# meta-pytorch/torchx

Measured on AMD Instinct MI355X. Metric: tokens_per_second, higher is better.
Workload: dtype bf16; 1 GPU; model=llama3_8b, global_batch=4, seq_len=4096, parallelism=dp1

## Files before the change

torchx_amd/ops/__init__.py:

```python

from __future__ import annotations

import importlib.util
import math
from pathlib import Path
from typing import Optional, Tuple

import torch

from . import reference

_SO = Path(__file__).resolve().parent / "_hip_ops.so"
_hip = None
_load_err: Optional[str] = None


def _load():
    global _hip, _load_err
    if _hip is not None:
        return _hip
    if not _SO.exists():
        _load_err = f"{_SO} not built (run torchx_amd/ops/build.py)"
        return None
    try:
# ... 144 lines not shown
        T, H = x2.shape
        dx = torch.empty_like(x2)
        single = T <= chunk
        dw_acc = None if single else torch.zeros_like(w, dtype=torch.float32)
        loss_sum = torch.zeros((), device=x2.device, dtype=torch.float32)
        inv_t = 1.0 / T
        gscale = torch.full((min(chunk, T),), inv_t, device=x2.device,
                            dtype=torch.float32)
        wt = (hip.transpose_bf16(w)
              if w.shape[0] % 64 == 0 and w.shape[1] % 64 == 0 else None)
        for s in range(0, T, chunk):
            e = min(T, s + chunk)
            x_c = x2[s:e]
            t_c = targets[s:e].contiguous()
            logits_c = x_c @ w.t()
            loss_c, lse_c = hip.ce_fwd(logits_c, t_c)
            loss_sum += loss_c.sum()
            dlog_c = hip.ce_bwd(logits_c, t_c, lse_c, gscale[:e - s])
            if wt is not None:
                torch.matmul(dlog_c, wt.t(), out=dx[s:e])
            else:
                torch.matmul(dlog_c, w, out=dx[s:e])
            if single:
                dw_acc = dlog_c.t() @ x_c
            else:
                dw_acc += dlog_c.t() @ x_c
        ctx.save_for_backward(dx, dw_acc)
        return loss_sum * inv_t

    @staticmethod
    def backward(ctx, gout: torch.Tensor):
        dx, dw_acc = ctx.saved_tensors
        if dw_acc.dtype == dx.dtype:
            dw = dw_acc * gout.to(dx.dtype)
        else:
            dw = (dw_acc * gout.to(torch.float32)).to(dx.dtype)
        dx = dx * gout.to(dx.dtype)
        return dx, dw, None, None


def fused_linear_cross_entropy(
    x: torch.Tensor, w: torch.Tensor, targets: torch.Tensor,
    chunk: int = 16384,
) -> torch.Tensor:
    H = x.shape[-1]
    x2 = x.reshape(-1, H)
    t = targets.reshape(-1)
    if _on_gpu(x):
        if torch.is_grad_enabled() and (x.requires_grad or w.requires_grad):
            return _FusedLinearCE.apply(x2.contiguous(), w, t, chunk)
        hip = hip_ops()
        x2 = x2.contiguous()
        T = x2.shape[0]
        loss_sum = torch.zeros((), device=x.device, dtype=torch.float32)
        for s in range(0, T, chunk):
            e = min(T, s + chunk)
            loss_c, _ = hip.ce_fwd(x2[s:e] @ w.t(), t[s:e].contiguous())
            loss_sum += loss_c.sum()
        return loss_sum / T
    return reference.cross_entropy(x2 @ w.t(), t)




class _FlashAttention(torch.autograd.Function):
    @staticmethod
    def forward(ctx, q: torch.Tensor, k: torch.Tensor, v: torch.Tensor,
                causal: bool, scale: float):
        o, lse = hip_ops().attn_fwd(
            q.contiguous(), k.contiguous(), v.contiguous(), scale, causal
        )
        ctx.save_for_backward(q, k, v, o, lse)
        ctx.causal = causal
        ctx.scale = scale
        return o

    @staticmethod
    def backward(ctx, dout: torch.Tensor):
        q, k, v, o, lse = ctx.saved_tensors
        dq, dk, dv = hip_ops().attn_bwd(
            q, k, v, o, dout.contiguous(), lse, ctx.scale, ctx.causal
        )
        return dq, dk, dv, None, None


def flash_attention(
    q: torch.Tensor, k: torch.Tensor, v: torch.Tensor,
    causal: bool = True, scale: Optional[float] = None,
) -> torch.Tensor:
    if scale is None:
        scale = 1.0 / math.sqrt(q.shape[-1])
    if _on_gpu(q):
        return _FlashAttention.apply(q, k, v, causal, scale)
    return reference.attention(q, k, v, causal=causal, scale=scale)




def adamw_step(
    p32: torch.Tensor, p16: torch.Tensor, grad: torch.Tensor,
    m: torch.Tensor, v: torch.Tensor, *, lr: float, beta1: float = 0.9,
    beta2: float = 0.95, eps: float = 1e-8, weight_decay: float = 0.1,
    step: int = 1,
) -> None:
    if p32.is_cuda:
        hip_ops().adamw_step(p32, p16, grad, m, v, lr, beta1, beta2, eps,
                             weight_decay, step)
    else:
        reference.adamw_step(p32, p16, grad, m, v, lr=lr, beta1=beta1,
                             beta2=beta2, eps=eps, weight_decay=weight_decay,
                             step=step)


def mfma_probe(a: torch.Tensor, b: torch.Tensor) -> torch.Tensor:
    return hip_ops().mfma_probe(a, b)




class _FastLinear(torch.autograd.Function):
    @staticmethod
    def forward(ctx, x: torch.Tensor, w: torch.Tensor):
        ctx.save_for_backward(x, w)
        return x @ w.t()

    @staticmethod
    def backward(ctx, dy: torch.Tensor):
        x, w = ctx.saved_tensors
        hip = hip_ops()
        wt = hip.transpose_bf16(w)
        dy2 = dy.reshape(-1, dy.shape[-1]).contiguous()
        x2 = x.reshape(-1, x.shape[-1])
        dx = (dy2 @ wt.t()).view_as(x)
        M, N = dy2.shape
        via_t = N <= 8192 and M % 64 == 0 and N % 64 == 0
        wg = w.grad if w.is_leaf else None
        if wg is not None and wg.is_contiguous():
            a = hip.transpose_bf16(dy2) if via_t else dy2.t()
            if getattr(w, "_wgrad_fresh", False):
                torch.matmul(a, x2, out=wg)
                w._wgrad_fresh = False
            else:
                wg.addmm_(a, x2)
            from torchx_amd.parallel.ddp import grad_ready

            grad_ready(w)
            return dx, None
        dw = (hip.transpose_bf16(dy2) @ x2) if via_t else (dy2.t() @ x2)
        return dx, dw


def fast_linear(x: torch.Tensor, w: torch.Tensor) -> torch.Tensor:
    if (x.is_cuda and w.dtype == torch.bfloat16
            and w.shape[0] % 64 == 0 and w.shape[1] % 64 == 0):
        return _FastLinear.apply(x, w)
    return torch.nn.functional.linear(x, w)




class _FusedAttentionQKV(torch.autograd.Function):
    @staticmethod
    def forward(ctx, qkv: torch.Tensor, cos: torch.Tensor, sin: torch.Tensor,
                Hq: int, Hkv: int, causal: bool, scale: float):
        hip = hip_ops()
        roped = hip.rope_qkv(qkv.contiguous(), cos, sin, Hq, Hkv, 1.0, False)
# ... 153 lines not shown
```

torchx_amd/ops/csrc/attention.hip:

```cpp
#include "common.h"

typedef __bf16 mbf16x8 __attribute__((ext_vector_type(8)));

#define HD 128
#define QBLK 32
#define KBLK 32
#define NWAVES 4
#define BLOCK_Q (QBLK * NWAVES)
#define BLOCK_K (KBLK * NWAVES)

__device__ __forceinline__ f32x16 mfma32(mbf16x8 a, mbf16x8 b, f32x16 c) {
  return __builtin_amdgcn_mfma_f32_32x32x16_bf16(a, b, c, 0, 0, 0);
}

__device__ __forceinline__ unsigned int pack_bf16x2(float a, float b) {
  unsigned int r;
  asm("v_cvt_pk_bf16_f32 %0, %1, %2" : "=v"(r) : "v"(a), "v"(b));
  return r;
}

__device__ __forceinline__ int c_row(int r, int half) {
  return (r & 3) + 8 * (r >> 2) + 4 * half;
}

// ... 301 lines not shown
      #pragma unroll
      for (int r = 0; r < 32; ++r) {
        sv[r] = __builtin_amdgcn_exp2f(sv[r] - m_run);
        row_sum += sv[r];
      }
      row_sum += __shfl_xor(row_sum, 32, 64);
      l_run += row_sum;

      mbf16x8 pf[4];
      cvals_to_frags(sv, hi, &pf[0], &pf[1]);
      cvals_to_frags(sv + 16, hi, &pf[2], &pf[3]);

      __builtin_amdgcn_s_setprio(1);
      #pragma unroll
      for (int dt = 0; dt < 4; ++dt) {
        #pragma unroll
        for (int ks = 0; ks < 4; ++ks) {
          acc_o[dt] = mfma32(nat_tr_frag(vcur, ks, dt), pf[ks], acc_o[dt]);
        }
      }
      __builtin_amdgcn_s_setprio(0);
    }

    if (has_next) {
      asm volatile("s_waitcnt vmcnt(0)");
      __syncthreads();
      char* tk = k0; k0 = k1; k1 = tk;
      char* tv = vcur; vcur = vnxt; vnxt = tv;
    }
  }

  if (!wave_active || q_row >= S) return;

  const float inv_l = (l_run > 0.f) ? 1.0f / l_run : 0.f;
  unsigned short* ob =
      o + (((long)b * S + q_row) * Hq + hq) * HD;
  #pragma unroll
  for (int dt = 0; dt < 4; ++dt) {
    #pragma unroll
    for (int g = 0; g < 4; ++g) {
      bf16x4_raw w;
      #pragma unroll
      for (int j = 0; j < 4; ++j) {
        w[j] = (short)f32_to_bf16(acc_o[dt][4 * g + j] * inv_l);
      }
      *(bf16x4_raw*)(ob + dt * 32 + 8 * g + 4 * (hi ? 1 : 0)) = w;
    }
  }
  if (!hi) {
    lse[((long)b * Hq + hq) * S + q_row] = (m_run + __log2f(l_run)) * LN2;
  }
}

__global__ void __launch_bounds__(256)
attn_bwd_pre_kernel(const unsigned short* __restrict__ dout,
                    const unsigned short* __restrict__ o,
                    float* __restrict__ delta,
                    long rows,
                    int S, int Hq) {
  const long row = (long)blockIdx.x * 16 + threadIdx.x / 16;
  if (row >= rows) return;
  const int sl = threadIdx.x & 15;
  const unsigned short* dp = dout + row * HD + sl * 8;
  const unsigned short* op = o + row * HD + sl * 8;
  ushort8 dv = *(const ushort8*)dp;
  ushort8 ov = *(const ushort8*)op;
  float acc = 0.f;
  #pragma unroll
  for (int j = 0; j < 8; ++j) {
    acc = fmaf(bf16_to_f32(dv[j]), bf16_to_f32(ov[j]), acc);
  }
  #pragma unroll
  for (int off = 8; off >= 1; off >>= 1) {
    acc += __shfl_down(acc, off, 16);
  }
  if (sl == 0) {
    const long b = row / ((long)S * Hq);
    const long s = (row / Hq) % S;
    const long h = row % Hq;
    delta[(b * Hq + h) * S + s] = acc;
  }
}

template <int TFKV>
__global__ void __launch_bounds__(256, 2)
attn_bwd_dq_kernel(const unsigned short* __restrict__ q,
                   const unsigned short* __restrict__ k,
                   const unsigned short* __restrict__ v,
                   const unsigned short* __restrict__ dout,
                   const float* __restrict__ lse,
                   const float* __restrict__ delta,
                   unsigned short* __restrict__ dq,
                   int B, int S, int Hq, int Hkv, float scale, int causal,
                   long q_rs, long kv_rs, long dq_rs) {
  __shared__ __align__(16) char smem[4 * (TFKV * 256)];
  char* kcur = smem;
  char* knxt = smem + TFKV * 256;
  char* vcur = smem + 2 * (TFKV * 256);
  char* vnxt = smem + 3 * (TFKV * 256);

  const int nqt = (S + BLOCK_Q - 1) / BLOCK_Q;
  const int G = Hq / Hkv;
  int b, hq, qt;
  map_block_fwd(B, Hq, Hkv, nqt, G, &b, &hq, &qt);
  const int hkv = hq / G;

  const int wave = threadIdx.x / 64;
  const int lane = threadIdx.x & 63;
  const bool hi = lane >= 32;
  const int qr = lane & 31;

  const long q_seq_stride = q_rs;
  const long kv_seq_stride = kv_rs;
  const unsigned short* qb = q + (long)b * S * q_seq_stride + (long)hq * HD;
  const unsigned short* kb = k + (long)b * S * kv_seq_stride + (long)hkv * HD;
  const unsigned short* vb = v + (long)b * S * kv_seq_stride + (long)hkv * HD;
  const unsigned short* dob =
      dout + ((long)b * S) * ((long)Hq * HD) + (long)hq * HD;

  const int q0_blk = qt * BLOCK_Q;
  const int qw0 = q0_blk + wave * QBLK;
  const long q_row = qw0 + qr;
  const bool wave_active = qw0 < S;
  const bool row_valid = q_row < S;

  mbf16x8 qfrag[8];
  float my_lse2 = 0.f, my_delta = 0.f;
  const long qrow_safe = row_valid ? q_row : (S - 1);
  const unsigned short* dop =
      dob + qrow_safe * ((long)Hq * HD) + (hi ? 8 : 0);
  {
    const unsigned short* qp = qb + qrow_safe * q_seq_stride + (hi ? 8 : 0);
    #pragma unroll
    for (int c = 0; c < 8; ++c) {
      qfrag[c] = __builtin_bit_cast(mbf16x8, *(const ushort8*)(qp + c * 16));
    }
    if (row_valid) {
      my_lse2 = lse[((long)b * Hq + hq) * S + q_row] * LOG2E;
      my_delta = delta[((long)b * Hq + hq) * S + q_row];
    }
  }

  f32x16 acc_dq[4] = {};
  const float sc2 = scale * LOG2E;

  const int kv_limit = causal ? min(S, q0_blk + BLOCK_Q) : S;
  const int ntiles = (kv_limit + TFKV - 1) / TFKV;
  const int qw_max = min(qw0 + QBLK - 1, S - 1);

  stage_k_glds<4, TFKV>(kb, 0, kv_seq_stride, S, kcur);
  stage_k_glds<4, TFKV>(vb, 0, kv_seq_stride, S, vcur);
  asm volatile("s_waitcnt vmcnt(0)");
  __syncthreads();

  for (int t = 0; t < ntiles; ++t) {
    const int kv0 = t * TFKV;
    const bool has_next = (t + 1) < ntiles;
    if (has_next) {
      stage_k_glds<4, TFKV>(kb, kv0 + TFKV, kv_seq_stride, S, knxt);
      stage_k_glds<4, TFKV>(vb, kv0 + TFKV, kv_seq_stride, S, vnxt);
    }

    const bool needed = wave_active && (!causal || kv0 <= qw_max);
    if (needed) {
      mbf16x8 dofrag[8];
      #pragma unroll
      for (int c = 0; c < 8; ++c) {
        dofrag[c] =
            __builtin_bit_cast(mbf16x8, *(const ushort8*)(dop + c * 16));
      }
      #pragma clang loop unroll(disable)
      for (int sb = 0; sb < TFKV / 32; ++sb) {
        if (causal && kv0 + 32 * sb > qw_max) break;
        f32x16 acc_s = {}, acc_dp = {};
        #pragma unroll
        for (int c = 0; c < 8; ++c) {
          acc_s = mfma32(kimg_frag(kcur, sb, c), qfrag[c], acc_s);
          acc_dp = mfma32(kimg_frag(vcur, sb, c), dofrag[c], acc_dp);
        }
        const int k0 = kv0 + 32 * sb;
        const bool mask_tile =
            (causal && k0 + 31 > qw0) || (k0 + 32 > S) || !row_valid;
        float ds[16];
        #pragma unroll
        for (int r = 0; r < 16; ++r) {
          float s2 = acc_s[r] * sc2;
          if (mask_tile) {
            const long kg = k0 + c_row(r, hi);
            if (kg >= S || !row_valid || (causal && kg > q_row)) {
              s2 = -3.0e38f;
            }
          }
          const float pr = __builtin_amdgcn_exp2f(s2 - my_lse2);
          ds[r] = scale * pr * (acc_dp[r] - my_delta);
        }
        mbf16x8 df0, df1;
        cvals_to_frags(ds, hi, &df0, &df1);
        #pragma unroll
        for (int dt = 0; dt < 4; ++dt) {
          acc_dq[dt] =
              mfma32(nat_tr_frag(kcur, 2 * sb, dt), df0, acc_dq[dt]);
          acc_dq[dt] =
              mfma32(nat_tr_frag(kcur, 2 * sb + 1, dt), df1, acc_dq[dt]);
        }
      }
    }

    if (has_next) {
      asm volatile("s_waitcnt vmcnt(0)");
      __syncthreads();
      char* tk = kcur; kcur = knxt; knxt = tk;
      char* tv = vcur; vcur = vnxt; vnxt = tv;
    }
  }

  if (!wave_active || !row_valid) return;
  unsigned short* dqb =
      dq + ((long)b * S + q_row) * dq_rs + (long)hq * HD;
  #pragma unroll
  for (int dt = 0; dt < 4; ++dt) {
    #pragma unroll
    for (int g = 0; g < 4; ++g) {
      bf16x4_raw w;
      #pragma unroll
      for (int j = 0; j < 4; ++j) {
        w[j] = (short)f32_to_bf16(acc_dq[dt][4 * g + j]);
      }
      *(bf16x4_raw*)(dqb + dt * 32 + 8 * g + 4 * (hi ? 1 : 0)) = w;
    }
  }
}

template <int TFKV = FKV>
__device__ __forceinline__ void stage_k_glds8(
    const unsigned short* __restrict__ kb, long kv0, long stride_elems,
    int S, char* kimg) {
  const int wave = threadIdx.x / 64;
  const int lane = threadIdx.x & 63;
  #pragma unroll
  for (int j = 0; j < TFKV / 32; ++j) {
    const int i = wave * (TFKV / 32) + j;
    const int row = i * 4 + (lane >> 4);
    const int colbyte = ((lane & 15) * 16) ^ ((row & 15) << 4);
    long srow = kv0 + row;
    if (srow >= S) srow = S - 1;
    const char* src = (const char*)(kb + srow * stride_elems) + colbyte;
    __builtin_amdgcn_global_load_lds(
        (const __attribute__((address_space(1))) unsigned int*)src,
        (__attribute__((address_space(3))) unsigned int*)(kimg + i * 1024),
        16, 0, 0);
  }
}


__device__ __forceinline__ void lds_nat_to_tr_own8(const char* nat,
                                                   char* tr_img) {
  const int wave = threadIdx.x / 64;
  const int lane = threadIdx.x & 63;
  #pragma unroll
  for (int pp = 0; pp < 2; ++pp) {
    const int c = wave * 128 + pp * 64 + lane;
    const int r = c >> 4, g = c & 15;
    const ushort8 v = *(const ushort8*)(
        nat + r * 256 + ((g * 16) ^ ((r & 15) << 4)));
    #pragma unroll
    for (int j = 0; j < 8; ++j) {
      const int d = 8 * g + j;
      const int gr = ((r >> 3) + vrot(d)) & 7;
      *(unsigned short*)(tr_img + d * 128 + gr * 16 + (r & 7) * 2) = v[j];
    }
  }
}

template <int TFKV>
__global__ void __launch_bounds__(512, 2)
attn_bwd_dkv_kernel(const unsigned short* __restrict__ q,
                    const unsigned short* __restrict__ k,
                    const unsigned short* __restrict__ v,
                    const unsigned short* __restrict__ dout,
                    const float* __restrict__ lse,
                    const float* __restrict__ delta,
                    unsigned short* __restrict__ dk,
                    unsigned short* __restrict__ dv,
                    int B, int S, int Hq, int Hkv, float scale, int causal,
                    long q_rs, long kv_rs, long dout_rs, long out_rs) {
  __shared__ __align__(16) char smem[4 * (TFKV * 256)];
  __shared__ float lse_buf[2][TFKV], del_buf[2][TFKV];
  char* qn_c = smem;
  char* don_c = smem + TFKV * 256;
  char* qn_n = smem + 2 * (TFKV * 256);
  char* don_n = smem + 3 * (TFKV * 256);

  const int nkt = (S + BLOCK_K - 1) / BLOCK_K;
  const int G = Hq / Hkv;
  int b, hkv, kt;
  {
    int bid = blockIdx.x;
    if (((B * Hkv) & 7) == 0) {
      const int xcd = bid & 7, slot = bid >> 3;
      const int g = (slot / nkt) * 8 + xcd;
      b = g / Hkv;
      hkv = g % Hkv;
      kt = slot % nkt;
    } else {
      b = bid / (Hkv * nkt);
      bid -= b * Hkv * nkt;
      hkv = bid / nkt;
      kt = bid % nkt;
    }
  }

  const int wave = threadIdx.x / 64;
  const bool is_dk = wave >= 4;
  const int lane = threadIdx.x & 63;
  const bool hi = lane >= 32;
  const int kr = lane & 31;

  const long q_seq_stride = q_rs;
  const long kv_seq_stride = kv_rs;
  const unsigned short* kb = k + (long)b * S * kv_seq_stride + (long)hkv * HD;
  const unsigned short* vb = v + (long)b * S * kv_seq_stride + (long)hkv * HD;

  const int kv0_blk = kt * BLOCK_K;
  const int kw0 = kv0_blk + (wave & 3) * KBLK;
  const long k_row = kw0 + kr;
  const bool wave_active = kw0 < S;
  const bool krow_valid = k_row < S;

  mbf16x8 kfrag[8], vfrag[8];
  {
    const long row = krow_valid ? k_row : (S - 1);
    const unsigned short* kp = kb + row * kv_seq_stride + (hi ? 8 : 0);
    const unsigned short* vp = vb + row * kv_seq_stride + (hi ? 8 : 0);
    #pragma unroll
    for (int c = 0; c < 8; ++c) {
      kfrag[c] = __builtin_bit_cast(mbf16x8, *(const ushort8*)(kp + c * 16));
      if (is_dk) {
        vfrag[c] =
            __builtin_bit_cast(mbf16x8, *(const ushort8*)(vp + c * 16));
      }
    }
  }

  f32x16 acc[4] = {};
  const float sc2 = scale * LOG2E;

  const int t0 = causal ? (kv0_blk / TFKV) : 0;
  const int nt = (S + TFKV - 1) / TFKV;
  const int nt_eff = nt - t0;
  const int total = G * nt_eff;

  auto head_q = [&](int gh) {
    return q + (long)b * S * q_seq_stride + (long)(hkv * G + gh) * HD;
  };
  auto head_do = [&](int gh) {
    return dout + (long)b * S * dout_rs + (long)(hkv * G + gh) * HD;
  };
  auto stage_lse = [&](int gh, int t, int buf) {
    const int hq_ = hkv * G + gh;
    const int q0_ = t * TFKV;
    if (threadIdx.x < TFKV) {
      const float* lse_b = lse + ((long)b * Hq + hq_) * S;
      const int qg = q0_ + threadIdx.x;
      lse_buf[buf][threadIdx.x] = (qg < S) ? lse_b[qg] * LOG2E : 0.f;
    } else if (threadIdx.x < 2 * TFKV) {
      const float* del_b = delta + ((long)b * Hq + hq_) * S;
      const int qg = q0_ + (threadIdx.x - TFKV);
      del_buf[buf][threadIdx.x - TFKV] = (qg < S) ? del_b[qg] : 0.f;
    }
  };

  stage_k_glds8<TFKV>(head_q(0), (long)t0 * TFKV, q_seq_stride, S, qn_c);
  stage_k_glds8<TFKV>(head_do(0), (long)t0 * TFKV, dout_rs, S, don_c);
  asm volatile("s_waitcnt vmcnt(0)");
  stage_lse(0, t0, 0);
  __syncthreads();

  const float* lse_cur = lse_buf[0];
  const float* del_cur = del_buf[0];
  int lse_nxt = 1;
  for (int idx = 0; idx < total; ++idx) {
    const int gh = idx / nt_eff;
    const int t = t0 + idx % nt_eff;
    const int q0 = t * TFKV;
    const int hq = hkv * G + gh;
    const bool has_next = (idx + 1) < total;
    const int ngh = (idx + 1) / nt_eff;
    const long nrow0 = (long)(t0 + (idx + 1) % nt_eff) * TFKV;
    if (has_next) {
      stage_k_glds8<TFKV>(head_q(ngh), nrow0, q_seq_stride, S, qn_n);
      stage_k_glds8<TFKV>(head_do(ngh), nrow0, dout_rs, S, don_n);
    }

    const bool needed =
        wave_active && (!causal || q0 + TFKV - 1 >= kw0);
    if (needed) {
      #pragma clang loop unroll(disable)
      for (int sb = 0; sb < TFKV / 32; ++sb) {
        if (causal && q0 + 32 * sb + 32 <= kw0) continue;
        f32x16 acc_s = {}, acc_dp = {};
        #pragma unroll
        for (int c = 0; c < 8; ++c) {
          acc_s = mfma32(kimg_frag(qn_c, sb, c), kfrag[c], acc_s);
          if (is_dk) {
            acc_dp = mfma32(kimg_frag(don_c, sb, c), vfrag[c], acc_dp);
          }
        }

        const int qs0 = q0 + 32 * sb;
        const bool mask_tile = (causal && qs0 < kw0 + 32)
                               || (qs0 + 32 > S) || !krow_valid;
        float cv[16];
        #pragma unroll
        for (int r = 0; r < 16; ++r) {
          const int ql = 32 * sb + c_row(r, hi);
          float s2 = acc_s[r] * sc2;
          if (mask_tile) {
            const long qg = q0 + ql;
            if (qg >= S || !krow_valid || (causal && k_row > qg)) {
              s2 = -3.0e38f;
            }
          }
          const float pr =
              __builtin_amdgcn_exp2f(s2 - lse_cur[ql]);
          cv[r] = is_dk ? scale * pr * (acc_dp[r] - del_cur[ql]) : pr;
        }

        mbf16x8 f0, f1;
        cvals_to_frags(cv, hi, &f0, &f1);

        const char* acc_img = is_dk ? qn_c : don_c;
        #pragma unroll
        for (int dt = 0; dt < 4; ++dt) {
          acc[dt] =
              mfma32(f0, nat_tr_frag(acc_img, 2 * sb, dt), acc[dt]);
          acc[dt] =
              mfma32(f1, nat_tr_frag(acc_img, 2 * sb + 1, dt), acc[dt]);
        }
      }
    }

    if (has_next) {
      asm volatile("s_waitcnt vmcnt(0)");
      stage_lse(ngh, t0 + (idx + 1) % nt_eff, lse_nxt);
      __syncthreads();
      lse_cur = lse_buf[lse_nxt];
      del_cur = del_buf[lse_nxt];
      lse_nxt ^= 1;
      char* tp;
      tp = qn_c; qn_c = qn_n; qn_n = tp;
      tp = don_c; don_c = don_n; don_n = tp;
    }
  }

  unsigned short* out = is_dk ? dk : dv;
  __syncthreads();
  float* tr = (float*)smem + wave * (32 * 36);
  if (wave_active) {
    #pragma unroll
    for (int dt = 0; dt < 4; ++dt) {
      __syncthreads();
      #pragma unroll
      for (int r = 0; r < 16; ++r) {
        tr[c_row(r, hi) * 36 + kr] = acc[dt][r];
      }
      __syncthreads();
      #pragma unroll
      for (int rep = 0; rep < 4; ++rep) {
        const int kk = kr;
        const int d0 = (hi ? 16 : 0) + rep * 4;
        if (kw0 + kk < S) {
          bf16x4_raw w;
          #pragma unroll
          for (int j = 0; j < 4; ++j) {
            w[j] = (short)f32_to_bf16(tr[kk * 36 + d0 + j]);
          }
          *(bf16x4_raw*)(out + ((long)b * S + kw0 + kk) * out_rs +
                         (long)hkv * HD + dt * 32 + d0) = w;
        }
      }
    }
  } else {
    #pragma unroll
    for (int i = 0; i < 8; ++i) __syncthreads();
  }
}

extern "C" void attn_fwd_launch(const void* q, const void* k, const void* v,
                                void* o, void* lse, int B, int S, int Hq,
                                int Hkv, float scale, int causal,
                                long q_rs, long kv_rs, hipStream_t stream) {
  static int fwd8 = -1;
  if (fwd8 < 0) {
    const char* e = getenv("TORCHX_AMD_FWD_8WAVE");
    fwd8 = (e && atoi(e)) ? 1 : 0;
  }
  if (fwd8 == 1) {
    const int nqt = (S + 8 * QBLK - 1) / (8 * QBLK);
    hipLaunchKernelGGL((attn_fwd_kernel<8>), dim3(B * Hq * nqt), dim3(512),
                       0, stream, (const unsigned short*)q,
                       (const unsigned short*)k, (const unsigned short*)v,
                       (unsigned short*)o, (float*)lse, B, S, Hq, Hkv,
                       scale, causal, q_rs, kv_rs);
  } else {
    const int nqt = (S + 4 * QBLK - 1) / (4 * QBLK);
    hipLaunchKernelGGL((attn_fwd_kernel<4>), dim3(B * Hq * nqt), dim3(256),
                       0, stream, (const unsigned short*)q,
                       (const unsigned short*)k, (const unsigned short*)v,
                       (unsigned short*)o, (float*)lse, B, S, Hq, Hkv,
                       scale, causal, q_rs, kv_rs);
  }
}

extern "C" void attn_bwd_launch(const void* q, const void* k, const void* v,
                                const void* o, const void* dout,
                                const void* lse, void* delta, void* dq,
                                void* dk, void* dv, int B, int S, int Hq,
                                int Hkv, float scale, int causal,
                                long q_rs, long kv_rs, long dqkv_q_rs,
                                long dqkv_kv_rs, hipStream_t stream) {
  const long rows = (long)B * S * Hq;
  hipLaunchKernelGGL(attn_bwd_pre_kernel, dim3((int)((rows + 15) / 16)),
                     dim3(256), 0, stream, (const unsigned short*)dout,
                     (const unsigned short*)o, (float*)delta, rows, S, Hq);
  const int nqt = (S + BLOCK_Q - 1) / BLOCK_Q;
  static int dq_fkv = -1;
  if (dq_fkv < 0) {
    const char* e = getenv("TORCHX_AMD_DQ_FKV");
    dq_fkv = (e && atoi(e) == 128) ? 128 : 64;
  }
  if (dq_fkv == 128 && S % 128 == 0) {
    hipLaunchKernelGGL((attn_bwd_dq_kernel<128>), dim3(B * Hq * nqt),
                       dim3(256), 0, stream, (const unsigned short*)q,
                       (const unsigned short*)k, (const unsigned short*)v,
                       (const unsigned short*)dout, (const float*)lse,
                       (const float*)delta, (unsigned short*)dq, B, S, Hq,
                       Hkv, scale, causal, q_rs, kv_rs, dqkv_q_rs);
  } else {
    hipLaunchKernelGGL((attn_bwd_dq_kernel<64>), dim3(B * Hq * nqt),
                       dim3(256), 0, stream, (const unsigned short*)q,
                       (const unsigned short*)k, (const unsigned short*)v,
                       (const unsigned short*)dout, (const float*)lse,
                       (const float*)delta, (unsigned short*)dq, B, S, Hq,
                       Hkv, scale, causal, q_rs, kv_rs, dqkv_q_rs);
  }
  const int nkt = (S + BLOCK_K - 1) / BLOCK_K;
  const long dout_rs = (long)Hq * HD;
  static int dkv_fkv = -1;
  if (dkv_fkv < 0) {
    const char* e = getenv("TORCHX_AMD_DKV_FKV");
    dkv_fkv = (e && atoi(e) == 64) ? 64 : 128;
  }
  if (dkv_fkv == 128 && S % 128 == 0) {
    hipLaunchKernelGGL((attn_bwd_dkv_kernel<128>), dim3(B * Hkv * nkt),
                       dim3(512), 0, stream, (const unsigned short*)q,
                       (const unsigned short*)k, (const unsigned short*)v,
                       (const unsigned short*)dout, (const float*)lse,
                       (const float*)delta, (unsigned short*)dk,
                       (unsigned short*)dv, B, S, Hq, Hkv,
                       scale, causal, q_rs, kv_rs, dout_rs, dqkv_kv_rs);
  } else {
    hipLaunchKernelGGL((attn_bwd_dkv_kernel<64>), dim3(B * Hkv * nkt),
                       dim3(512), 0, stream, (const unsigned short*)q,
                       (const unsigned short*)k, (const unsigned short*)v,
                       (const unsigned short*)dout, (const float*)lse,
                       (const float*)delta, (unsigned short*)dk,
                       (unsigned short*)dv, B, S, Hq, Hkv,
                       scale, causal, q_rs, kv_rs, dout_rs, dqkv_kv_rs);
  }
}
```

torchx_amd/ops/csrc/bindings.cpp:

```cpp
#include <torch/extension.h>
#include <c10/hip/HIPStream.h>

#include <hip/hip_runtime.h>

extern "C" {
void rope_launch(const void*, void*, const void*, const void*, long, int, int,
                 int, float, hipStream_t);
void swiglu_fwd_launch(const void*, const void*, void*, long, hipStream_t);
void swiglu_bwd_launch(const void*, const void*, const void*, void*, void*,
                       long, hipStream_t);
void rmsnorm_fwd_launch(const void*, const void*, void*, void*, long, int,
                        float, hipStream_t);
void rmsnorm_bwd_launch(const void*, const void*, const void*, const void*,
                        void*, void*, void*, long, int, hipStream_t);
long rmsnorm_bwd_dw_chunks(long);
void adamw_launch(void*, void*, const void*, void*, void*, long, float, float,
                  float, float, float, float, float, hipStream_t);
void ce_fwd_launch(const void*, const void*, void*, void*, long, int,
                   hipStream_t);
void ce_bwd_launch(const void*, const void*, const void*, const void*, void*,
                   long, int, hipStream_t);
void attn_fwd_launch(const void*, const void*, const void*, void*, void*, int,
                     int, int, int, float, int, long, long, hipStream_t);
void attn_bwd_launch(const void*, const void*, const void*, const void*,
                     const void*, const void*, void*, void*, void*, void*,
                     int, int, int, int, float, int, long, long, long, long,
                     hipStream_t);
void rope_qkv_launch(const void*, void*, const void*, const void*, long, int,
                     long, int, float, hipStream_t);
void swiglu_gu_fwd_launch(const void*, void*, long, long, hipStream_t);
void swiglu_gu_bwd_launch(const void*, const void*, void*, long, long,
                          hipStream_t);
void mfma_probe_launch(const void*, const void*, void*, hipStream_t);
void mfma_probe_tr_launch(const void*, const void*, void*, void*,
                          hipStream_t);
void fp8_cast_transpose_launch(const void*, void*, void*, void*,
                               const void*, long, long, int, hipStream_t);
void transpose_bf16_launch(const void*, void*, long, long, hipStream_t);
void decode_attn_launch(const void*, const void*, const void*, void*,
                        const void*, int, int, int, int, int, int, float,
                        hipStream_t);
void gemv_bf16_launch(const void*, const void*, void*, int, int, int,
                      hipStream_t);
void decode_attn_split_launch(const void*, const void*, const void*, void*,
                              void*, void*, const void*, int, int, int, int,
                              int, int, int, float, hipStream_t);
void decode_rope_cache_launch(const void*, void*, void*, void*, const void*,
                              const void*, const void*, int, int, int, int,
                              int, int, hipStream_t);
void rmsnorm_res_launch(const void*, const void*, const void*, void*, void*,
                        long, int, float, hipStream_t);
void gemv_swiglu_launch(const void*, const void*, void*, int, int, int,
                        hipStream_t);
}

namespace {

hipStream_t cur_stream() {
  return c10::hip::getCurrentHIPStream().stream();
}

void check_bf16(const at::Tensor& t, const char* name) {
  TORCH_CHECK(t.is_cuda(), name, " must be on GPU");
  TORCH_CHECK(t.scalar_type() == at::kBFloat16, name, " must be bf16");
  TORCH_CHECK(t.is_contiguous(), name, " must be contiguous");
}

void check_f32(const at::Tensor& t, const char* name) {
  TORCH_CHECK(t.is_cuda(), name, " must be on GPU");
  TORCH_CHECK(t.scalar_type() == at::kFloat, name, " must be f32");
  TORCH_CHECK(t.is_contiguous(), name, " must be contiguous");
}

}

std::vector<at::Tensor> rmsnorm_fwd(at::Tensor x, at::Tensor w, double eps) {
  check_bf16(x, "x");
  check_bf16(w, "w");
  const long H = x.size(-1);
  TORCH_CHECK(H % 2048 == 0 && H <= 8192, "rmsnorm: H must be k*2048, <=8192");
  const long rows = x.numel() / H;
  auto y = at::empty_like(x);
  auto invrms = at::empty({rows}, x.options().dtype(at::kFloat));
  rmsnorm_fwd_launch(x.data_ptr(), w.data_ptr(), y.data_ptr(),
                     invrms.data_ptr(), rows, (int)H, (float)eps,
                     cur_stream());
  return {y, invrms};
}

std::vector<at::Tensor> rmsnorm_bwd(at::Tensor dy, at::Tensor x, at::Tensor w,
                                    at::Tensor invrms) {
  check_bf16(dy, "dy");
  check_bf16(x, "x");
  const long H = x.size(-1);
  TORCH_CHECK(H % 2048 == 0 && H <= 8192, "rmsnorm: H must be k*2048, <=8192");
  const long rows = x.numel() / H;
  auto dx = at::empty_like(x);
  auto dw = at::empty({H}, x.options().dtype(at::kFloat));
  auto dw_part = at::empty({rmsnorm_bwd_dw_chunks(rows), H}, dw.options());
  rmsnorm_bwd_launch(dy.data_ptr(), x.data_ptr(), w.data_ptr(),
                     invrms.data_ptr(), dx.data_ptr(), dw.data_ptr(),
                     dw_part.data_ptr(), rows, (int)H, cur_stream());
  return {dx, dw};
}

at::Tensor rope(at::Tensor x, at::Tensor cos_t, at::Tensor sin_t, long heads,
                double sign) {
  check_bf16(x, "x");
  check_f32(cos_t, "cos");
  check_f32(sin_t, "sin");
// ... 4 lines not shown
  auto y = at::empty_like(x);
  rope_launch(x.data_ptr(), y.data_ptr(), cos_t.data_ptr(), sin_t.data_ptr(),
              rows, (int)D, (int)heads, (int)S, (float)sign, cur_stream());
  return y;
}

at::Tensor swiglu_fwd(at::Tensor g, at::Tensor u) {
  check_bf16(g, "g");
  check_bf16(u, "u");
  auto out = at::empty_like(g);
  swiglu_fwd_launch(g.data_ptr(), u.data_ptr(), out.data_ptr(), g.numel(),
                    cur_stream());
  return out;
}

std::vector<at::Tensor> swiglu_bwd(at::Tensor dout, at::Tensor g,
                                   at::Tensor u) {
  check_bf16(dout, "dout");
  auto dg = at::empty_like(g);
  auto du = at::empty_like(u);
  swiglu_bwd_launch(dout.data_ptr(), g.data_ptr(), u.data_ptr(), dg.data_ptr(),
                    du.data_ptr(), g.numel(), cur_stream());
  return {dg, du};
}

void adamw_step(at::Tensor p32, at::Tensor p16, at::Tensor g, at::Tensor m,
                at::Tensor v, double lr, double beta1, double beta2,
                double eps, double wd, long step) {
  check_f32(p32, "p32");
  check_bf16(p16, "p16");
  check_bf16(g, "g");
  const long n = p32.numel();
  TORCH_CHECK(n % 4 == 0, "adamw: n must be a multiple of 4");
  const float bc1 = 1.0f - powf((float)beta1, (float)step);
  const float bc2 = 1.0f - powf((float)beta2, (float)step);
  adamw_launch(p32.data_ptr(), p16.data_ptr(), g.data_ptr(), m.data_ptr(),
               v.data_ptr(), n, (float)lr, (float)beta1, (float)beta2,
               (float)eps, (float)wd, bc1, bc2, cur_stream());
}

std::vector<at::Tensor> ce_fwd(at::Tensor logits, at::Tensor targets) {
  check_bf16(logits, "logits");
  TORCH_CHECK(targets.scalar_type() == at::kLong, "targets must be int64");
  const long V = logits.size(-1);
  const long T = logits.numel() / V;
  auto loss = at::empty({T}, logits.options().dtype(at::kFloat));
  auto lse = at::empty({T}, logits.options().dtype(at::kFloat));
  ce_fwd_launch(logits.data_ptr(), targets.data_ptr(), loss.data_ptr(),
                lse.data_ptr(), T, (int)V, cur_stream());
  return {loss, lse};
}

at::Tensor ce_bwd(at::Tensor logits, at::Tensor targets, at::Tensor lse,
                  at::Tensor gscale) {
  check_bf16(logits, "logits");
  check_f32(lse, "lse");
  check_f32(gscale, "gscale");
  const long V = logits.size(-1);
  const long T = logits.numel() / V;
  auto dlogits = at::empty_like(logits);
  ce_bwd_launch(logits.data_ptr(), targets.data_ptr(), lse.data_ptr(),
                gscale.data_ptr(), dlogits.data_ptr(), T, (int)V,
                cur_stream());
  return dlogits;
}

std::vector<at::Tensor> attn_fwd(at::Tensor q, at::Tensor k, at::Tensor v,
                                 double scale, bool causal) {
  check_bf16(q, "q");
  check_bf16(k, "k");
  check_bf16(v, "v");
  const int B = q.size(0), S = q.size(1), Hq = q.size(2), D = q.size(3);
  const int Hkv = k.size(2);
  TORCH_CHECK(D == 128, "attention: head_dim must be 128");
  TORCH_CHECK(Hq % Hkv == 0, "attention: Hq must be a multiple of Hkv");
  auto o = at::empty_like(q);
  auto lse = at::empty({B, Hq, S}, q.options().dtype(at::kFloat));
  attn_fwd_launch(q.data_ptr(), k.data_ptr(), v.data_ptr(), o.data_ptr(),
                  lse.data_ptr(), B, S, Hq, Hkv, (float)scale, causal ? 1 : 0,
                  (long)Hq * 128, (long)Hkv * 128, cur_stream());
  return {o, lse};
}

std::vector<at::Tensor> attn_bwd(at::Tensor q, at::Tensor k, at::Tensor v,
                                 at::Tensor o, at::Tensor dout, at::Tensor lse,
                                 double scale, bool causal) {
  check_bf16(dout, "dout");
  const int B = q.size(0), S = q.size(1), Hq = q.size(2);
  const int Hkv = k.size(2);
  auto dq = at::empty_like(q);
  auto dk = at::empty_like(k);
  auto dv = at::empty_like(v);
  auto delta = at::empty({B, Hq, S}, q.options().dtype(at::kFloat));
  attn_bwd_launch(q.data_ptr(), k.data_ptr(), v.data_ptr(), o.data_ptr(),
                  dout.data_ptr(), lse.data_ptr(), delta.data_ptr(),
                  dq.data_ptr(), dk.data_ptr(), dv.data_ptr(), B, S, Hq, Hkv,
                  (float)scale, causal ? 1 : 0, (long)Hq * 128,
                  (long)Hkv * 128, (long)Hq * 128, (long)Hkv * 128,
                  cur_stream());
  return {dq, dk, dv};
}

std::vector<at::Tensor> attn_fwd_qkv(at::Tensor qkv, long Hq, long Hkv,
                                     double scale, bool causal) {
  check_bf16(qkv, "qkv");
  const int B = qkv.size(0), S = qkv.size(1);
  const long rs = (Hq + 2 * Hkv) * 128;
  TORCH_CHECK(qkv.size(2) == rs, "qkv last dim mismatch");
  auto o = at::empty({B, S, Hq, 128}, qkv.options());
  auto lse = at::empty({B, Hq, S}, qkv.options().dtype(at::kFloat));
  const unsigned short* base = (const unsigned short*)qkv.data_ptr();
  attn_fwd_launch(base, base + Hq * 128, base + (Hq + Hkv) * 128,
                  o.data_ptr(), lse.data_ptr(), B, S, (int)Hq, (int)Hkv,
                  (float)scale, causal ? 1 : 0, rs, rs, cur_stream());
  return {o, lse};
}

at::Tensor attn_bwd_qkv(at::Tensor qkv, at::Tensor o, at::Tensor dout,
                        at::Tensor lse, long Hq, long Hkv, double scale,
                        bool causal) {
  check_bf16(dout, "dout");
  const int B = qkv.size(0), S = qkv.size(1);
  const long rs = (Hq + 2 * Hkv) * 128;
  auto dqkv = at::empty_like(qkv);
  auto delta = at::empty({B, Hq, S}, qkv.options().dtype(at::kFloat));
  const unsigned short* base = (const unsigned short*)qkv.data_ptr();
  unsigned short* dbase = (unsigned short*)dqkv.data_ptr();
  attn_bwd_launch(base, base + Hq * 128, base + (Hq + Hkv) * 128,
                  o.data_ptr(), dout.data_ptr(), lse.data_ptr(),
                  delta.data_ptr(), dbase, dbase + Hq * 128,
                  dbase + (Hq + Hkv) * 128, B, S, (int)Hq, (int)Hkv,
                  (float)scale, causal ? 1 : 0, rs, rs, rs, rs,
                  cur_stream());
  return dqkv;
}

at::Tensor rope_qkv(at::Tensor x, at::Tensor cos_t, at::Tensor sin_t,
                    long Hq, long Hkv, double sign, bool inplace) {
  check_bf16(x, "x");
  check_f32(cos_t, "cos");
  check_f32(sin_t, "sin");
  const int B = x.size(0), S = x.size(1);
  const long rs = (Hq + 2 * Hkv) * 128;
  TORCH_CHECK(x.size(2) == rs, "qkv last dim mismatch");
  at::Tensor y = inplace ? x : at::empty_like(x);
  rope_qkv_launch(x.data_ptr(), y.data_ptr(), cos_t.data_ptr(),
                  sin_t.data_ptr(), (long)B * S, (int)(Hq + Hkv), rs, S,
                  (float)sign, cur_stream());
  if (!inplace) {
    const long v0 = (Hq + Hkv) * 128;
    y.narrow(2, v0, Hkv * 128).copy_(x.narrow(2, v0, Hkv * 128));
  }
  return y;
}

at::Tensor swiglu_gu_fwd(at::Tensor gu) {
  check_bf16(gu, "gu");
  const long twoI = gu.size(-1);
  TORCH_CHECK(twoI % 16 == 0, "gu last dim must be 2I, I % 8 == 0");
  const long I = twoI / 2;
  const long rows = gu.numel() / twoI;
  auto sizes = gu.sizes().vec();
  sizes.back() = I;
  auto out = at::empty(sizes, gu.options());
  swiglu_gu_fwd_launch(gu.data_ptr(), out.data_ptr(), rows, I, cur_stream());
  return out;
}

at::Tensor swiglu_gu_bwd(at::Tensor dout, at::Tensor gu) {
  check_bf16(dout, "dout");
  const long twoI = gu.size(-1);
  const long I = twoI / 2;
  const long rows = gu.numel() / twoI;
  auto dgu = at::empty_like(gu);
  swiglu_gu_bwd_launch(dout.data_ptr(), gu.data_ptr(), dgu.data_ptr(), rows,
                       I, cur_stream());
  return dgu;
}

std::vector<at::Tensor> fp8_cast_transpose(at::Tensor x, at::Tensor scale,
                                           bool e5m2) {
  check_bf16(x, "x");
  check_f32(scale, "scale");
  const long C = x.size(-1);
  const long R = x.numel() / C;
  TORCH_CHECK(R % 8 == 0 && C % 8 == 0, "fp8 cast: dims must be 8-aligned");
  auto dt = e5m2 ? at::kFloat8_e5m2 : at::kFloat8_e4m3fn;
  auto out = at::empty({R, C}, x.options().dtype(dt));
  auto out_t = at::empty({C, R}, x.options().dtype(dt));
  auto amax = at::zeros({1}, x.options().dtype(at::kFloat));
  fp8_cast_transpose_launch(x.data_ptr(), out.data_ptr(), out_t.data_ptr(),
                            amax.data_ptr(), scale.data_ptr(), R, C,
                            e5m2 ? 1 : 0, cur_stream());
  return {out, out_t, amax};
}

at::Tensor transpose_bf16(at::Tensor x) {
  check_bf16(x, "x");
  TORCH_CHECK(x.dim() == 2, "transpose_bf16: 2D only");
  const long R = x.size(0), C = x.size(1);
  TORCH_CHECK(R % 64 == 0 && C % 64 == 0,
              "transpose_bf16: dims must be multiples of 64");
  auto out = at::empty({C, R}, x.options());
  transpose_bf16_launch(x.data_ptr(), out.data_ptr(), R, C, cur_stream());
  return out;
}

at::Tensor decode_attn(at::Tensor q, at::Tensor kc, at::Tensor vc, long L,
                       double scale) {
  check_bf16(q, "q");
  check_bf16(kc, "kc");
  check_bf16(vc, "vc");
  const int B = q.size(0), Hq = q.size(1);
  const int T = kc.size(1), Hkv = kc.size(2);
  TORCH_CHECK(q.size(2) == 128 && kc.size(3) == 128, "head_dim must be 128");
// ... 87 lines not shown
  TORCH_CHECK(kc.size(3) == 128 && cos_t.size(1) == 64,
              "head_dim must be 128");
  const long nh = qkv.size(1) / 128;
  const int Hq = (int)nh - 2 * Hkv;
  TORCH_CHECK(Hq >= 1 && qkv.size(1) == nh * 128, "qkv width mismatch");
  const void* pd = nullptr;
  int per_row = 0;
  if (pos_dev.has_value()) {
    TORCH_CHECK(pos_dev->scalar_type() == at::kInt &&
                    (pos_dev->numel() == 1 || pos_dev->numel() == B),
                "pos_dev must be an int32 scalar or [B] tensor");
    TORCH_CHECK(pos_dev->is_contiguous(), "pos_dev must be contiguous");
    pd = pos_dev->data_ptr();
    per_row = pos_dev->numel() == B && B > 1 ? 1 : 0;
  } else {
    TORCH_CHECK(pos >= 0 && pos < T, "pos out of cache range");
    TORCH_CHECK(pos < cos_t.size(0), "pos beyond rope table");
  }
  auto q = at::empty({B, (long)Hq, 128}, qkv.options());
  decode_rope_cache_launch(qkv.data_ptr(), q.data_ptr(), kc.data_ptr(),
                           vc.data_ptr(), cos_t.data_ptr(), sin_t.data_ptr(),
                           pd, B, Hq, Hkv, T, (int)pos, per_row,
                           cur_stream());
  return q;
}

std::vector<at::Tensor> rmsnorm_res(at::Tensor x,
                                    c10::optional<at::Tensor> res,
                                    at::Tensor w, double eps) {
  check_bf16(x, "x");
  check_bf16(w, "w");
  const long H = x.size(-1);
  TORCH_CHECK(H % 2048 == 0 && H <= 8192, "rmsnorm: H must be k*2048, <=8192");
  const long R = x.numel() / H;
  auto y = at::empty_like(x);
  at::Tensor s = x;
  const void* rp = nullptr;
  void* sp = nullptr;
  if (res.has_value()) {
    check_bf16(*res, "res");
    TORCH_CHECK(res->sizes() == x.sizes(), "res shape mismatch");
    s = at::empty_like(x);
    rp = res->data_ptr();
    sp = s.data_ptr();
  }
  rmsnorm_res_launch(x.data_ptr(), rp, w.data_ptr(), sp, y.data_ptr(), R,
                     (int)H, (float)eps, cur_stream());
  return {s, y};
}

std::vector<at::Tensor> mfma_probe_tr(at::Tensor a, at::Tensor b) {
  check_bf16(a, "a");
  check_bf16(b, "b");
  TORCH_CHECK(a.size(0) == 32 && a.size(1) == 16, "a must be [32,16]");
  TORCH_CHECK(b.size(0) == 16 && b.size(1) == 32, "b must be [16,32]");
  auto c = at::empty({32, 32}, a.options().dtype(at::kFloat));
  auto raw = at::empty({64, 8}, a.options());
  mfma_probe_tr_launch(a.data_ptr(), b.data_ptr(), c.data_ptr(),
                       raw.data_ptr(), cur_stream());
  return {c, raw};
}

at::Tensor mfma_probe(at::Tensor a, at::Tensor b) {
  check_bf16(a, "a");
  check_bf16(b, "b");
  TORCH_CHECK(a.size(0) == 32 && a.size(1) == 16, "a must be [32,16]");
  TORCH_CHECK(b.size(0) == 16 && b.size(1) == 32, "b must be [16,32]");
  auto c = at::empty({32, 32}, a.options().dtype(at::kFloat));
  mfma_probe_launch(a.data_ptr(), b.data_ptr(), c.data_ptr(), cur_stream());
  return c;
}

PYBIND11_MODULE(TORCH_EXTENSION_NAME, m) {
  m.def("rmsnorm_fwd", &rmsnorm_fwd);
  m.def("rmsnorm_bwd", &rmsnorm_bwd);
  m.def("rope", &rope);
  m.def("swiglu_fwd", &swiglu_fwd);
  m.def("swiglu_bwd", &swiglu_bwd);
  m.def("adamw_step", &adamw_step);
  m.def("ce_fwd", &ce_fwd);
  m.def("ce_bwd", &ce_bwd);
  m.def("attn_fwd", &attn_fwd);
  m.def("attn_bwd", &attn_bwd);
  m.def("attn_fwd_qkv", &attn_fwd_qkv);
  m.def("attn_bwd_qkv", &attn_bwd_qkv);
  m.def("rope_qkv", &rope_qkv);
  m.def("swiglu_gu_fwd", &swiglu_gu_fwd);
  m.def("swiglu_gu_bwd", &swiglu_gu_bwd);
  m.def("fp8_cast_transpose", &fp8_cast_transpose);
  m.def("mfma_probe", &mfma_probe);
  m.def("mfma_probe_tr", &mfma_probe_tr);
  m.def("transpose_bf16", &transpose_bf16);
  m.def("decode_attn", &decode_attn);
  m.def("decode_attn_dev", &decode_attn_dev);
  m.def("gemv_bf16", &gemv_bf16);
  m.def("gemv_swiglu_bf16", &gemv_swiglu_bf16);
  m.def("decode_rope_cache", &decode_rope_cache,
        py::arg("qkv"), py::arg("kc"), py::arg("vc"), py::arg("cos"),
        py::arg("sin"), py::arg("pos") = 0,
        py::arg("pos_dev") = c10::nullopt);
  m.def("rmsnorm_res", &rmsnorm_res,
        py::arg("x"), py::arg("res"), py::arg("w"), py::arg("eps"));
}
```

Before: 19580 tokens/s.

## Stream dS from dKV kernel to a scratch buffer and compute dQ from it

```diff
diff --git a/torchx_amd/ops/__init__.py b/torchx_amd/ops/__init__.py
--- a/torchx_amd/ops/__init__.py
+++ b/torchx_amd/ops/__init__.py
@@ -250,6 +250,14 @@
             q, k, v, o, dout.contiguous(), lse, ctx.scale, ctx.causal
         )
         return dq, dk, dv, None, None
+
+
+def set_attn_bwd_dq_mode(mode: str) -> None:
+    hip_ops().set_attn_bwd_dq_mode(mode)
+
+
+def get_attn_bwd_dq_mode() -> str:
+    return hip_ops().get_attn_bwd_dq_mode()
 
 
 def flash_attention(
diff --git a/torchx_amd/ops/csrc/attention.hip b/torchx_amd/ops/csrc/attention.hip
--- a/torchx_amd/ops/csrc/attention.hip
+++ b/torchx_amd/ops/csrc/attention.hip
@@ -407,6 +407,18 @@
   }
 }
 
+#define DS_IMG_BYTES 2048
+
+__host__ __device__ __forceinline__ long ds_qt_base(int qt, int nqt,
+                                                    int causal) {
+  return causal ? 2L * qt * (qt + 1) : 4L * qt * nqt;
+}
+
+extern "C" long attn_bwd_ds_bytes(int B, int S, int Hq, int causal) {
+  const int nqt = (S + BLOCK_Q - 1) / BLOCK_Q;
+  return (long)B * Hq * ds_qt_base(nqt, nqt, causal) * 4 * DS_IMG_BYTES;
+}
+
 template <int TFKV>
 __global__ void __launch_bounds__(256, 2)
 attn_bwd_dq_kernel(const unsigned short* __restrict__ q,
@@ -556,6 +568,134 @@
   }
 }
 
+__device__ __forceinline__ mbf16x8 ds_tr_frag(const char* img, int ks) {
+  const int lane = threadIdx.x & 63;
+  const int j = lane & 15;
+  const int r_lo = ks * 16 + ((lane >> 5) * 8) + (j >> 2);
+  const int cb = ((lane >> 4) & 1) * 32 + (j & 3) * 8;
+  short4_v lo = __builtin_amdgcn_ds_read_tr16_b64_v4i16(
+      (lds_s4p)(img + r_lo * 64 + cb));
+  short4_v hi = __builtin_amdgcn_ds_read_tr16_b64_v4i16(
+      (lds_s4p)(img + (r_lo + 4) * 64 + cb));
+  uint2_v ul = __builtin_bit_cast(uint2_v, lo);
+  uint2_v uh = __builtin_bit_cast(uint2_v, hi);
+  uint4_v u = {ul[0], ul[1], uh[0], uh[1]};
+  return __builtin_bit_cast(mbf16x8, u);
+}
+
+__global__ void __launch_bounds__(256, 2)
+attn_bwd_dq_stream_kernel(const unsigned short* __restrict__ k,
+                          const char* __restrict__ ds,
+                          unsigned short* __restrict__ dq,
+                          int B, int S, int Hq, int Hkv, int causal,
+                          long kv_rs, long dq_rs, int heavy_first) {
+  __shared__ __align__(16) char smem[2 * KIMG_BYTES + 16 * DS_IMG_BYTES];
+
+  const int nqt = (S + BLOCK_Q - 1) / BLOCK_Q;
+  const int G = Hq / Hkv;
+  int b, hq, qt;
+  map_block_fwd(B, Hq, Hkv, nqt, G, &b, &hq, &qt);
+  if (heavy_first) qt = nqt - 1 - qt;
+  const int hkv = hq / G;
+
+  const int wave = threadIdx.x / 64;
+  const int lane = threadIdx.x & 63;
+  const bool hi = lane >= 32;
+
+  char* kcur = smem;
+  char* knxt = smem + KIMG_BYTES;
+  char* dcur = smem + 2 * KIMG_BYTES + wave * (2 * DS_IMG_BYTES);
+  char* dnxt = dcur + 8 * DS_IMG_BYTES;
+
+  const unsigned short* kb = k + (long)b * S * kv_rs + (long)hkv * HD;
+  const int q0_blk = qt * BLOCK_Q;
+  const int qw0 = q0_blk + wave * QBLK;
+  const long q_row = qw0 + (lane & 31);
+  const bool wave_active = qw0 < S;
+  const int k_last =
+      !wave_active ? -1 : (causal ? qw0 : ((S - 1) / KBLK) * KBLK);
+  const char* ds_w =
+      ds + ((((long)b * Hq + hq) * ds_qt_base(nqt, nqt, causal) +
+             ds_qt_base(qt, nqt, causal)) * 4 + wave) * DS_IMG_BYTES +
+      lane * 16;
+
+  auto stage_ds = [&](int kv0, char* dst) {
+    #pragma unroll
+    for (int sb = 0; sb < FKV / 32; ++sb) {
+      const int k0 = kv0 + 32 * sb;
+      if (k0 <= k_last) {
+        const char* src = ds_w + (long)(k0 / KBLK) * (4 * DS_IMG_BYTES);
+        #pragma unroll
+        for (int i = 0; i < 2; ++i) {
+          __builtin_amdgcn_global_load_lds(
+              (const __attribute__((address_space(1))) unsigned int*)(
+                  src + i * 1024),
+              (__attribute__((address_space(3))) unsigned int*)(
+                  dst + sb * DS_IMG_BYTES + i * 1024),
+              16, 0, 0);
+        }
+      }
+    }
+  };
+
+  f32x16 acc_dq[4] = {};
+
+  const int kv_limit = causal ? min(S, q0_blk + BLOCK_Q) : S;
+  const int ntiles = (kv_limit + FKV - 1) / FKV;
+
+  stage_k_glds<4, FKV>(kb, 0, kv_rs, S, kcur);
+  stage_ds(0, dcur);
+  asm volatile("s_waitcnt vmcnt(0)");
+  __syncthreads();
+
+  for (int t = 0; t < ntiles; ++t) {
+    const int kv0 = t * FKV;
+    const bool has_next = (t + 1) < ntiles;
+    if (has_next) {
+      stage_k_glds<4, FKV>(kb, kv0 + FKV, kv_rs, S, knxt);
+      stage_ds(kv0 + FKV, dnxt);
+    }
+
+    if (kv0 <= k_last) {
+      #pragma unroll
+      for (int sb = 0; sb < FKV / 32; ++sb) {
+        if (kv0 + 32 * sb > k_last) break;
+        const mbf16x8 df0 = ds_tr_frag(dcur + sb * DS_IMG_BYTES, 0);
+        const mbf16x8 df1 = ds_tr_frag(dcur + sb * DS_IMG_BYTES, 1);
+        #pragma unroll
+        for (int dt = 0; dt < 4; ++dt) {
+          acc_dq[dt] =
+              mfma32(nat_tr_frag(kcur, 2 * sb, dt), df0, acc_dq[dt]);
+          acc_dq[dt] =
+              mfma32(nat_tr_frag(kcur, 2 * sb + 1, dt), df1, acc_dq[dt]);
+        }
+      }
+    }
+
+    if (has_next) {
+      asm volatile("s_waitcnt vmcnt(0)");
+      __syncthreads();
+      char* tk = kcur; kcur = knxt; knxt = tk;
+      char* td = dcur; dcur = dnxt; dnxt = td;
+    }
+  }
+
+  if (!wave_active || q_row >= S) return;
+  unsigned short* dqb = dq + ((long)b * S + q_row) * dq_rs + (long)hq * HD;
+  #pragma unroll
+  for (int dt = 0; dt < 4; ++dt) {
+    #pragma unroll
+    for (int g = 0; g < 4; ++g) {
+      bf16x4_raw w;
+      #pragma unroll
+      for (int j = 0; j < 4; ++j) {
+        w[j] = (short)f32_to_bf16(acc_dq[dt][4 * g + j]);
+      }
+      *(bf16x4_raw*)(dqb + dt * 32 + 8 * g + 4 * (hi ? 1 : 0)) = w;
+    }
+  }
+}
+
 template <int TFKV = FKV>
 __device__ __forceinline__ void stage_k_glds8(
     const unsigned short* __restrict__ kb, long kv0, long stride_elems,
@@ -607,6 +747,7 @@
                     const float* __restrict__ delta,
                     unsigned short* __restrict__ dk,
                     unsigned short* __restrict__ dv,
+                    char* __restrict__ ds,
                     int B, int S, int Hq, int Hkv, float scale, int causal,
                     long q_rs, long kv_rs, long dout_rs, long out_rs) {
   __shared__ __align__(16) char smem[4 * (TFKV * 256)];
@@ -674,6 +815,12 @@
   const int nt = (S + TFKV - 1) / TFKV;
   const int nt_eff = nt - t0;
   const int total = G * nt_eff;
+
+  const bool ds_on = is_dk && ds != nullptr;
+  const int ds_nqt = (S + BLOCK_Q - 1) / BLOCK_Q;
+  const long ds_plane = ds_qt_base(ds_nqt, ds_nqt, causal);
+  const long ds_lane = (long)(kw0 / KBLK) * (4 * DS_IMG_BYTES) + kr * 64 +
+                       (hi ? 16 : 0);
 
   auto head_q = [&](int gh) {
     return q + (long)b * S * q_seq_stride + (long)(hkv * G + gh) * HD;
@@ -719,7 +866,10 @@
 
     const bool needed =
         wave_active && (!causal || q0 + TFKV - 1 >= kw0);
+    int n_ds = 0;
     if (needed) {
+      char* ds_head = ds + ((long)b * Hq + hq) * ds_plane * (4 * DS_IMG_BYTES)
+                      + ds_lane;
       #pragma clang loop unroll(disable)
       for (int sb = 0; sb < TFKV / 32; ++sb) {
         if (causal && q0 + 32 * sb + 32 <= kw0) continue;
@@ -761,12 +911,27 @@
               mfma32(f0, nat_tr_frag(acc_img, 2 * sb, dt), acc[dt]);
           acc[dt] =
               mfma32(f1, nat_tr_frag(acc_img, 2 * sb + 1, dt), acc[dt]);
+          if (dt == 0) {
+            __builtin_amdgcn_sched_barrier(0);
+            if (ds_on && qs0 < S) {
+              char* p = ds_head +
+                        (ds_qt_base(qs0 / BLOCK_Q, ds_nqt, causal) * 4 +
+                         ((qs0 / QBLK) & 3)) * DS_IMG_BYTES;
+              *(uint4_v*)p = __builtin_bit_cast(uint4_v, f0);
+              *(uint4_v*)(p + 32) = __builtin_bit_cast(uint4_v, f1);
+              n_ds = 2;
+            }
+          }
         }
       }
     }
 
     if (has_next) {
-      asm volatile("s_waitcnt vmcnt(0)");
+      if (n_ds) {
+        asm volatile("s_waitcnt vmcnt(2)" ::: "memory");
+      } else {
+        asm volatile("s_waitcnt vmcnt(0)" ::: "memory");
+      }
       stage_lse(ngh, t0 + (idx + 1) % nt_eff, lse_nxt);
       __syncthreads();
       lse_cur = lse_buf[lse_nxt];
@@ -840,15 +1005,51 @@
 extern "C" void attn_bwd_launch(const void* q, const void* k, const void* v,
                                 const void* o, const void* dout,
                                 const void* lse, void* delta, void* dq,
-                                void* dk, void* dv, int B, int S, int Hq,
-                                int Hkv, float scale, int causal,
+                                void* dk, void* dv, void* ds, int B, int S,
+                                int Hq, int Hkv, float scale, int causal,
                                 long q_rs, long kv_rs, long dqkv_q_rs,
                                 long dqkv_kv_rs, hipStream_t stream) {
   const long rows = (long)B * S * Hq;
   hipLaunchKernelGGL(attn_bwd_pre_kernel, dim3((int)((rows + 15) / 16)),
                      dim3(256), 0, stream, (const unsigned short*)dout,
                      (const unsigned short*)o, (float*)delta, rows, S, Hq);
+  const int nkt = (S + BLOCK_K - 1) / BLOCK_K;
+  const long dout_rs = (long)Hq * HD;
+  static int dkv_fkv = -1;
+  if (dkv_fkv < 0) {
+    const char* e = getenv("TORCHX_AMD_DKV_FKV");
+    dkv_fkv = (e && atoi(e) == 64) ? 64 : 128;
+  }
+  if (dkv_fkv == 128 && S % 128 == 0) {
+    hipLaunchKernelGGL((attn_bwd_dkv_kernel<128>), dim3(B * Hkv * nkt),
+                       dim3(512), 0, stream, (const unsigned short*)q,
+                       (const unsigned short*)k, (const unsigned short*)v,
+                       (const unsigned short*)dout, (const float*)lse,
+                       (const float*)delta, (unsigned short*)dk,
+                       (unsigned short*)dv, (char*)ds, B, S, Hq, Hkv,
+                       scale, causal, q_rs, kv_rs, dout_rs, dqkv_kv_rs);
+  } else {
+    hipLaunchKernelGGL((attn_bwd_dkv_kernel<64>), dim3(B * Hkv * nkt),
+                       dim3(512), 0, stream, (const unsigned short*)q,
+                       (const unsigned short*)k, (const unsigned short*)v,
+                       (const unsigned short*)dout, (const float*)lse,
+                       (const float*)delta, (unsigned short*)dk,
+                       (unsigned short*)dv, (char*)ds, B, S, Hq, Hkv,
+                       scale, causal, q_rs, kv_rs, dout_rs, dqkv_kv_rs);
+  }
   const int nqt = (S + BLOCK_Q - 1) / BLOCK_Q;
+  if (ds != nullptr) {
+    static int heavy_first = -1;
+    if (heavy_first < 0) {
+      const char* e = getenv("TORCHX_AMD_DQ_HEAVY_FIRST");
+      heavy_first = (e && atoi(e) == 0) ? 0 : 1;
+    }
+    hipLaunchKernelGGL(attn_bwd_dq_stream_kernel, dim3(B * Hq * nqt),
+                       dim3(256), 0, stream, (const unsigned short*)k,
+                       (const char*)ds, (unsigned short*)dq, B, S, Hq, Hkv,
+                       causal, kv_rs, dqkv_q_rs, heavy_first);
+    return;
+  }
   static int dq_fkv = -1;
   if (dq_fkv < 0) {
     const char* e = getenv("TORCHX_AMD_DQ_FKV");
@@ -869,28 +1070,4 @@
                        (const float*)delta, (unsigned short*)dq, B, S, Hq,
                        Hkv, scale, causal, q_rs, kv_rs, dqkv_q_rs);
   }
-  const int nkt = (S + BLOCK_K - 1) / BLOCK_K;
-  const long dout_rs = (long)Hq * HD;
-  static int dkv_fkv = -1;
-  if (dkv_fkv < 0) {
-    const char* e = getenv("TORCHX_AMD_DKV_FKV");
-    dkv_fkv = (e && atoi(e) == 64) ? 64 : 128;
-  }
-  if (dkv_fkv == 128 && S % 128 == 0) {
-    hipLaunchKernelGGL((attn_bwd_dkv_kernel<128>), dim3(B * Hkv * nkt),
-                       dim3(512), 0, stream, (const unsigned short*)q,
-                       (const unsigned short*)k, (const unsigned short*)v,
-                       (const unsigned short*)dout, (const float*)lse,
-                       (const float*)delta, (unsigned short*)dk,
-                       (unsigned short*)dv, B, S, Hq, Hkv,
-                       scale, causal, q_rs, kv_rs, dout_rs, dqkv_kv_rs);
-  } else {
-    hipLaunchKernelGGL((attn_bwd_dkv_kernel<64>), dim3(B * Hkv * nkt),
-                       dim3(512), 0, stream, (const unsigned short*)q,
-                       (const unsigned short*)k, (const unsigned short*)v,
-                       (const unsigned short*)dout, (const float*)lse,
-                       (const float*)delta, (unsigned short*)dk,
-                       (unsigned short*)dv, B, S, Hq, Hkv,
-                       scale, causal, q_rs, kv_rs, dout_rs, dqkv_kv_rs);
-  }
-}
+}
diff --git a/torchx_amd/ops/csrc/bindings.cpp b/torchx_amd/ops/csrc/bindings.cpp
--- a/torchx_amd/ops/csrc/bindings.cpp
+++ b/torchx_amd/ops/csrc/bindings.cpp
@@ -24,8 +24,9 @@
                      int, int, int, float, int, long, long, hipStream_t);
 void attn_bwd_launch(const void*, const void*, const void*, const void*,
                      const void*, const void*, void*, void*, void*, void*,
-                     int, int, int, int, float, int, long, long, long, long,
-                     hipStream_t);
+                     void*, int, int, int, int, float, int, long, long, long,
+                     long, hipStream_t);
+long attn_bwd_ds_bytes(int, int, int, int);
 void rope_qkv_launch(const void*, void*, const void*, const void*, long, int,
                      long, int, float, hipStream_t);
 void swiglu_gu_fwd_launch(const void*, void*, long, long, hipStream_t);
@@ -196,6 +197,37 @@
   return {o, lse};
 }
 
+int g_dq_stream = -1;
+
+bool dq_stream_mode() {
+  if (g_dq_stream < 0) {
+    const char* e = getenv("TORCHX_AMD_DQ_MODE");
+    g_dq_stream = (e && std::string(e) == "recompute") ? 0 : 1;
+  }
+  return g_dq_stream == 1;
+}
+
+void set_attn_bwd_dq_mode(const std::string& mode) {
+  TORCH_CHECK(mode == "stream" || mode == "recompute",
+              "attn bwd dq mode must be 'stream' or 'recompute', got '",
+              mode, "'");
+  g_dq_stream = (mode == "stream") ? 1 : 0;
+}
+
+std::string get_attn_bwd_dq_mode() {
+  return dq_stream_mode() ? "stream" : "recompute";
+}
+
+constexpr long kDsScratchCapBytes = 8L << 30;
+
+at::Tensor alloc_ds_scratch(const at::Tensor& like, int B, int S, int Hq,
+                            bool causal) {
+  if (!dq_stream_mode()) return at::Tensor();
+  const long bytes = attn_bwd_ds_bytes(B, S, Hq, causal ? 1 : 0);
+  if (bytes > kDsScratchCapBytes) return at::Tensor();
+  return at::empty({bytes}, like.options().dtype(at::kByte));
+}
+
 std::vector<at::Tensor> attn_bwd(at::Tensor q, at::Tensor k, at::Tensor v,
                                  at::Tensor o, at::Tensor dout, at::Tensor lse,
                                  double scale, bool causal) {
@@ -206,9 +238,11 @@
   auto dk = at::empty_like(k);
   auto dv = at::empty_like(v);
   auto delta = at::empty({B, Hq, S}, q.options().dtype(at::kFloat));
+  auto ds = alloc_ds_scratch(q, B, S, Hq, causal);
   attn_bwd_launch(q.data_ptr(), k.data_ptr(), v.data_ptr(), o.data_ptr(),
                   dout.data_ptr(), lse.data_ptr(), delta.data_ptr(),
-                  dq.data_ptr(), dk.data_ptr(), dv.data_ptr(), B, S, Hq, Hkv,
+                  dq.data_ptr(), dk.data_ptr(), dv.data_ptr(),
+                  ds.defined() ? ds.data_ptr() : nullptr, B, S, Hq, Hkv,
                   (float)scale, causal ? 1 : 0, (long)Hq * 128,
                   (long)Hkv * 128, (long)Hq * 128, (long)Hkv * 128,
                   cur_stream());
@@ -238,13 +272,15 @@
   const long rs = (Hq + 2 * Hkv) * 128;
   auto dqkv = at::empty_like(qkv);
   auto delta = at::empty({B, Hq, S}, qkv.options().dtype(at::kFloat));
+  auto ds = alloc_ds_scratch(qkv, B, S, (int)Hq, causal);
   const unsigned short* base = (const unsigned short*)qkv.data_ptr();
   unsigned short* dbase = (unsigned short*)dqkv.data_ptr();
   attn_bwd_launch(base, base + Hq * 128, base + (Hq + Hkv) * 128,
                   o.data_ptr(), dout.data_ptr(), lse.data_ptr(),
                   delta.data_ptr(), dbase, dbase + Hq * 128,
-                  dbase + (Hq + Hkv) * 128, B, S, (int)Hq, (int)Hkv,
-                  (float)scale, causal ? 1 : 0, rs, rs, rs, rs,
+                  dbase + (Hq + Hkv) * 128,
+                  ds.defined() ? ds.data_ptr() : nullptr, B, S, (int)Hq,
+                  (int)Hkv, (float)scale, causal ? 1 : 0, rs, rs, rs, rs,
                   cur_stream());
   return dqkv;
 }
@@ -498,6 +534,8 @@
   m.def("ce_bwd", &ce_bwd);
   m.def("attn_fwd", &attn_fwd);
   m.def("attn_bwd", &attn_bwd);
+  m.def("set_attn_bwd_dq_mode", &set_attn_bwd_dq_mode);
+  m.def("get_attn_bwd_dq_mode", &get_attn_bwd_dq_mode);
   m.def("attn_fwd_qkv", &attn_fwd_qkv);
   m.def("attn_bwd_qkv", &attn_bwd_qkv);
   m.def("rope_qkv", &rope_qkv);
```

Result: faster. 20100 tokens/s, median of 6 (+2.6%).
